# Tesla-Albert/Hybrid-Grid-for-Hexagonal-and-Rectangular-Image-Processing

Measured on AMD Instinct MI355X. Metric: Mpix/s rect→hex→rect+hexconv, 4K batch=128, 1/2/4/8 GPU; %HBM roofline, higher is better.
Workload: dtype bf16

## Files before the change

hybrid-grid-for-hexagonal-and-rectangular-image-processing_amd/csrc/fused4.hip:

```cpp
#include <climits>
#include <cmath>
#include <cstdlib>

#include "fused_kernel.h"

namespace hg {

#ifndef F4_RB_
#define F4_RB_ 30
#endif
#ifndef F4_PD
#define F4_PD 2
#endif
#ifndef F4_WPS
#define F4_WPS 29
#endif
#ifndef F4_ORDER
#define F4_ORDER 0
#endif
#ifndef F4_WPE
#define F4_WPE 3
#endif
#ifndef F4_REV
#define F4_REV 1
#endif
constexpr int F4_GW = 4, F4_THREADS = 256;
constexpr int F4_HL = 8, F4_OWN = 240;
constexpr int F4_RB = F4_RB_;
static_assert(F4_RB % 6 == 0 && F4_RB > 0, "bands are whole 6-step blocks");

typedef unsigned f4_u2 __attribute__((ext_vector_type(2)));

__device__ __forceinline__ void f4_unpack(f4_u2 r, fu_f2& a, fu_f2& b, unsigned hi16) {
    a = fu_f2{__builtin_bit_cast(float, r.x << 16), __builtin_bit_cast(float, r.x & hi16)};
    b = fu_f2{__builtin_bit_cast(float, r.y << 16), __builtin_bit_cast(float, r.y & hi16)};
}

template <int OP>
__global__ __launch_bounds__(F4_THREADS) __attribute__((amdgpu_waves_per_eu(F4_WPE)))
void k_fused4(const __bf16* __restrict__ x, const float* __restrict__ kern,
              const float* __restrict__ bias, __bf16* __restrict__ y, FusedGeom F) {
    constexpr int C = 3, O = 3;
    constexpr int PD = F4_PD;
    static_assert(PD >= 1 && PD <= 4, "raw ring: rows k+2 .. k+1+PD in flight in 6 slots");
    constexpr int RB = F4_RB, NLUT = RB + 2;
    __shared__ float4 lut_all[F4_GW][NLUT];
    const int lane = threadIdx.x & 63;
    const int wslot = __builtin_amdgcn_readfirstlane(threadIdx.x >> 6);
    float4* const lut = lut_all[wslot];
    const int64_t blk = (int64_t)xcd_swizzle(blockIdx.x, gridDim.x);
    const int ngrp = (F.nwin + F4_GW - 1) / F4_GW;
    const int grp = (int)(F4_ORDER == 1 ? (blk / F.nband) % ngrp : blk % ngrp);
    const int band = (int)(F4_ORDER == 1 ? blk % F.nband : (blk / ngrp) % F.nband);
    const int64_t b = blk / ((int64_t)ngrp * F.nband);
    if (b >= F.B) return;
    const int win = grp * F4_GW + wslot;
    const int W0 = win * F4_OWN - F4_HL;
    const int ce = W0 + 4 * lane;
    const int s0 = band * RB;
    const int s1 = min(s0 + RB, F.h2);
    const bool up = F4_REV && (band & 1) && s1 - s0 == RB;

    for (int e = lane; e < NLUT; e += 64) {
        const int r = s0 - 1 + e;
        float4 t = {0.f, 0.f, 0.f, 0.f};
        if (r >= 0 && r < F.h1) {
            const double i_ = axis_at(F.rxs, r) + (double)(F.h - 1) * 0.5;
            const int in = (int)i_;
            const double f = i_ - (double)(float)in;
            const float w0 = (in >= 0 && in < F.h) ? (float)(1.0 - f) : 0.f;
            const float w1 = (in + 1 >= 0 && in + 1 < F.h) ? (float)f : 0.f;
            if (in == r - 1) { t.x = w0; t.y = w1; }
            else if (in == r) { t.y = w0; t.z = w1; }
        }
        lut[e] = t;
    }
    __builtin_amdgcn_s_waitcnt(0xc07f);
    __builtin_amdgcn_wave_barrier();
    int rc;
    {
        bool has_a = false, has_c = false;
        for (int e = lane; e < NLUT; e += 64) {
            const float4 t = lut[e];
            has_a |= t.x != 0.f;
            has_c |= t.z != 0.f;
        }
        const bool any_a = __builtin_amdgcn_ballot_w64(has_a) != 0;
        const bool any_c = __builtin_amdgcn_ballot_w64(has_c) != 0;
        rc = !any_c ? 1 : (!any_a ? 2 : 0);
    }

    float we[2][3], wo[2][3];
#pragma unroll
    for (int k = 0; k < 2; ++k)
#pragma unroll
        for (int s = 0; s < 2; ++s) {
            float* wr = s ? wo[k] : we[k];
            wr[0] = wr[1] = wr[2] = 0.f;
            const int q = ce + 2 * k + s;
            if (q >= 0 && q < F.w1) {
                const double j_ = axis_at(F.rys, q) + (double)(F.w - 1) * 0.5;
                const int jn = (int)j_;
                const double jf = j_ - (double)(float)jn;
#pragma unroll
                for (int kk = -1; kk <= 1; ++kk) {
                    const bool in_w = q + kk >= 0 && q + kk < F.w;
                    if (kk == jn - q && in_w) wr[kk + 1] += (float)(1.0 - jf);
                    if (kk == jn + 1 - q && in_w) wr[kk + 1] += (float)jf;
                }
            }
#pragma unroll
            for (int t = 0; t < 3; ++t) wr[t] *= 0.75f;
        }
    const bool any_l = __builtin_amdgcn_ballot_w64(we[0][0] != 0.f || wo[0][0] != 0.f ||
                                                   we[1][0] != 0.f || wo[1][0] != 0.f) != 0;
    const bool any_r = __builtin_amdgcn_ballot_w64(we[0][2] != 0.f || wo[0][2] != 0.f ||
                                                   we[1][2] != 0.f || wo[1][2] != 0.f) != 0;
    const int cd = !any_r ? 1 : (!any_l ? 2 : 0);

    const bool own = lane >= F4_HL / 4 && lane < (F4_HL + F4_OWN) / 4 && ce >= 0 && ce < F.w2 &&
                     win < F.nwin;

    const int64_t cstride = (int64_t)F.h * F.w, ostride = (int64_t)F.h2 * F.w2;
    const __amdgpu_buffer_rsrc_t xrs = __builtin_amdgcn_make_buffer_rsrc(
        (void*)(x + b * C * cstride), (short)0, (int)(C * cstride * 2), 0x00020000);
    const __amdgpu_buffer_rsrc_t yrs = __builtin_amdgcn_make_buffer_rsrc(
        (void*)(y + b * O * ostride), (short)0, (int)(O * ostride * 2), 0x00020000);
    const int lc = min(max(ce, 0), F.w - 4);
    const unsigned xoff = (unsigned)lc * 2u;
    const unsigned yoff = own ? (unsigned)ce * 2u : 0x80000000u;
    const unsigned xplane = (unsigned)(cstride * 2), yplane = (unsigned)(ostride * 2);
    const unsigned xrow = (unsigned)F.w * 2u, yrow = (unsigned)F.w2 * 2u;
    auto row_off = [&](int r) -> unsigned {
        return (unsigned)__builtin_amdgcn_readfirstlane((int)((unsigned)min(max(r, 0), F.h - 1) * xrow));
    };

    int vz = 0;
    asm volatile("" : "+v"(vz));
    constexpr int NW = O * C * 7, NWP = (NW + 1) / 2;
    constexpr int NWS = F4_WPS < NWP ? F4_WPS : NWP;
    float wk[NW];
#pragma unroll
    for (int i = 0; i < NW; ++i) wk[i] = kern[i + (i / 2 < NWS ? 0 : vz)];
    fu_f2 wkp[NWP];
#pragma unroll
    for (int i = 0; i < NWP; ++i) {
        wkp[i] = fu_f2{wk[2 * i], 2 * i + 1 < NW ? wk[2 * i + 1] : 0.f};
        if (i >= NWS) asm volatile("" : "+v"(wkp[i]));
    }
    float bv[O];
#pragma unroll
    for (int o = 0; o < O; ++o) bv[o] = bias ? bias[o + vz] * 0.75f : 0.f;
    fu_f2 bvp[2];
#pragma unroll
    for (int i = 0; i < 2; ++i) {
        bvp[i] = fu_f2{bv[2 * i], 2 * i + 1 < O ? bv[2 * i + 1] : 0.f};
        asm volatile("" : "+v"(bvp[i]));
    }
    float c13 = 1.f / 3.f;
    asm volatile("" : "+v"(c13));
    const float wn_f = (ce + 4 < F.w2) ? c13 : 0.f;
    const float wp_f = (ce - 1 >= 0) ? c13 : 0.f;
    unsigned hi16 = 0xffff0000u;
    asm volatile("" : "+v"(hi16));

    auto run = [&](auto CDc, auto RCc, auto UPc) {
        constexpr int CD = decltype(CDc)::value;
        constexpr int RC = decltype(RCc)::value;
        constexpr bool UP = decltype(UPc)::value;
        auto row = [&](int k) { return UP ? s1 - 1 - k : s0 + k; };
        auto lut_e = [&](int j) { return UP ? RB - j : j + 1; };
        f4_u2 raw[6][C];
        fu_f2 XA[3][C], XB[3][C];
        fu_f2 ZA[3][O], ZB[3][O];

        auto issue = [&](auto SLc, int r, bool live = true) {
            constexpr int SL = decltype(SLc)::value;
            const unsigned so = row_off(r);
            const unsigned vo = live ? xoff : 0x80000000u;
#pragma unroll
            for (int c = 0; c < C; ++c) raw[SL][c] = __builtin_amdgcn_raw_buffer_load_b64(xrs, vo, so + c * xplane, 0);
        };
        auto convert = [&](auto RSc, auto XSc) {
            constexpr int RS = decltype(RSc)::value, XS = decltype(XSc)::value;
#pragma unroll
            for (int c = 0; c < C; ++c) f4_unpack(raw[RS][c], XA[XS][c], XB[XS][c], hi16);
        };

        auto urow = [&](auto PHc, float4 L, auto CENc, auto BELc) {
            constexpr int PH = decltype(PHc)::value;
            constexpr bool CEN = decltype(CENc)::value, BEL = decltype(BELc)::value;
            constexpr int S0 = fu_mod(PH, 3), S1 = fu_mod(PH + 1, 3), S2 = fu_mod(PH + 2, 3);
            constexpr int XM = UP ? S2 : S0, XQ = UP ? S0 : S2;
            constexpr int PB = UP ? fu_mod(PH + 1, 2) : fu_mod(PH, 2), PC = 1 - PB;
            constexpr int TN = UP ? 5 : 0, TD = UP ? 0 : 5;
            const fu_f2 Lxy = {L.x, L.y}, Lzw = {L.z, L.w};
            fu_sfor<0, C>([&](auto Cc) {
                constexpr int c = decltype(Cc)::value;
                float ue[2], uo[2];
                auto vblend = [&](const fu_f2 (&X)[3][C]) {
                    if constexpr (RC == 1) return fu_pfma<1, false>(Lxy, X[S1][c], fu_pmul<0>(Lxy, X[XM][c]));
                    else if constexpr (RC == 2) return fu_pfma<0, false>(Lzw, X[XQ][c], fu_pmul<1>(Lxy, X[S1][c]));
                    else return fu_pfma<0, false>(Lzw, X[XQ][c], fu_pfma<1, false>(Lxy, X[S1][c], fu_pmul<0>(Lxy, X[XM][c])));
                };
                const fu_f2 VA = vblend(XA), VB = vblend(XB);
                if constexpr (CD == 1) {
                    ue[0] = fmaf(we[0][1], VA.x, we[0][0] * f_prev(VB.y));
                    uo[0] = fmaf(wo[0][1], VA.y, wo[0][0] * VA.x);
                    ue[1] = fmaf(we[1][1], VB.x, we[1][0] * VA.y);
                    uo[1] = fmaf(wo[1][1], VB.y, wo[1][0] * VB.x);
                } else if constexpr (CD == 2) {
                    ue[0] = fmaf(we[0][2], VA.y, we[0][1] * VA.x);
                    uo[0] = fmaf(wo[0][2], VB.x, wo[0][1] * VA.y);
                    ue[1] = fmaf(we[1][2], VB.y, we[1][1] * VB.x);
                    uo[1] = fmaf(wo[1][2], f_next(VA.x), wo[1][1] * VB.y);
                } else {
                    const float pl = f_prev(VB.y), nx = f_next(VA.x);
                    ue[0] = fmaf(we[0][2], VA.y, fmaf(we[0][1], VA.x, we[0][0] * pl));
                    uo[0] = fmaf(wo[0][2], VB.x, fmaf(wo[0][1], VA.y, wo[0][0] * VA.x));
                    ue[1] = fmaf(we[1][2], VB.y, fmaf(we[1][1], VB.x, we[1][0] * VA.y));
                    uo[1] = fmaf(wo[1][2], nx, fmaf(wo[1][1], VB.y, wo[1][0] * VB.x));
                }
                const float nue = f_next(ue[0]);
                const fu_f2 U0[2] = {fu_f2{ue[0], uo[0]}, fu_f2{ue[1], uo[1]}};
                const fu_f2 U1[2] = {fu_f2{uo[0], ue[1]}, fu_f2{uo[1], nue}};
                const fu_f2 Um[2] = {fu_f2{f_prev(uo[1]), ue[0]}, fu_f2{uo[0], ue[1]}};
                const fu_f2 U2[2] = {U0[1], fu_f2{nue, OP == 0 ? f_next(uo[0]) : 0.f}};
                fu_sfor<0, O>([&](auto OOc) {
                    constexpr int o = decltype(OOc)::value;
                    constexpr int j0 = (o * C + c) * 7;
                    auto tapk = [&](auto Tc, fu_f2& zA, fu_f2& zB, int par) {
                        constexpr int j = j0 + decltype(Tc)::value;
                        constexpr bool WS = (j >> 1) < NWS;
                        const int s = fu_tap_shift(decltype(Tc)::value, par, OP);
                        const fu_f2 aA = s == -1 ? Um[0] : (s == 0 ? U0[0] : (s == 1 ? U1[0] : U2[0]));
                        const fu_f2 aB = s == -1 ? Um[1] : (s == 0 ? U0[1] : (s == 1 ? U1[1] : U2[1]));
                        zA = fu_pfma<j & 1, WS>(wkp[j >> 1], aA, zA);
                        zB = fu_pfma<j & 1, WS>(wkp[j >> 1], aB, zB);
                    };
                    if constexpr (c == 0) {
                        constexpr int jb = j0 + TN;
                        constexpr bool WS = (jb >> 1) < NWS;
                        const int s = fu_tap_shift(TN, PB, OP);
                        const fu_f2 aA = s == -1 ? Um[0] : (s == 0 ? U0[0] : (s == 1 ? U1[0] : U2[0]));
                        const fu_f2 aB = s == -1 ? Um[1] : (s == 0 ? U0[1] : (s == 1 ? U1[1] : U2[1]));
                        ZA[S2][o] = fu_pfma_b<jb & 1, o & 1, WS>(wkp[jb >> 1], aA, bvp[o >> 1]);
                        ZB[S2][o] = fu_pfma_b<jb & 1, o & 1, WS>(wkp[jb >> 1], aB, bvp[o >> 1]);
                    } else {
                        tapk(IC<TN>{}, ZA[S2][o], ZB[S2][o], PB);
                    }
                    tapk(IC<TN + 1>{}, ZA[S2][o], ZB[S2][o], PB);
                    if constexpr (CEN) {
                        tapk(IC<2>{}, ZA[S1][o], ZB[S1][o], PC);
                        tapk(IC<3>{}, ZA[S1][o], ZB[S1][o], PC);
                        tapk(IC<4>{}, ZA[S1][o], ZB[S1][o], PC);
                    }
                    if constexpr (BEL) {
                        tapk(IC<TD>{}, ZA[S0][o], ZB[S0][o], PB);
                        tapk(IC<TD + 1>{}, ZA[S0][o], ZB[S0][o], PB);
                    }
                });
            });
        };

        auto out_row = [&](auto PHc, int k) {
            constexpr int PH = decltype(PHc)::value;
            constexpr int S0 = PH % 3;
            constexpr int PAR = UP ? (PH + 1) & 1 : PH & 1;
            const unsigned so = (unsigned)__builtin_amdgcn_readfirstlane((int)((unsigned)row(k) * yrow));
#pragma unroll
            for (int o = 0; o < O; ++o) {
                const fu_f2 zA = ZA[S0][o], zB = ZB[S0][o];
                float o0, o1, o2, o3;
                if constexpr (PAR == 0) {
                    o0 = fmaf(c13, zA.y, zA.x);
                    o1 = fmaf(c13, zB.x, zA.y);
                    o2 = fmaf(c13, zB.y, zB.x);
                    o3 = fmaf(wn_f, f_next(zA.x), zB.y);
                } else {
                    o0 = fmaf(wp_f, f_prev(zB.y), zA.x);
                    o1 = fmaf(c13, zA.x, zA.y);
                    o2 = fmaf(c13, zA.y, zB.x);
                    o3 = fmaf(c13, zB.x, zB.y);
                }
                typedef __bf16 t2v __attribute__((ext_vector_type(2)));
                const f4_u2 v = {__builtin_bit_cast(unsigned, t2v{(__bf16)o0, (__bf16)o1}),
                                 __builtin_bit_cast(unsigned, t2v{(__bf16)o2, (__bf16)o3})};
                __builtin_amdgcn_raw_buffer_store_b64(v, yrs, yoff, so + o * yplane, 0);
            }
        };

        {
            f4_u2 t0[C], t1[C], t2[C];
            const unsigned o0 = row_off(row(-2)), o1 = row_off(row(-1)), o2 = row_off(row(0));
#pragma unroll
            for (int c = 0; c < C; ++c) {
                t0[c] = __builtin_amdgcn_raw_buffer_load_b64(xrs, xoff, o0 + c * xplane, 0);
                t1[c] = __builtin_amdgcn_raw_buffer_load_b64(xrs, xoff, o1 + c * xplane, 0);
                t2[c] = __builtin_amdgcn_raw_buffer_load_b64(xrs, xoff, o2 + c * xplane, 0);
            }
            issue(IC<1>{}, row(1));
#pragma unroll
            for (int i = 0; i < PD; ++i) {
                if (i == 0) issue(IC<2>{}, row(2));
                if (i == 1) issue(IC<3>{}, row(3));
                if (i == 2) issue(IC<4>{}, row(4));
                if (i == 3) issue(IC<5>{}, row(5));
            }
#pragma unroll
            for (int c = 0; c < C; ++c) {
                f4_unpack(t0[c], XA[1][c], XB[1][c], hi16);
                f4_unpack(t1[c], XA[2][c], XB[2][c], hi16);
                f4_unpack(t2[c], XA[0][c], XB[0][c], hi16);
            }
        }
        urow(IC<-2>{}, lut[lut_e(-1)], std::false_type{}, std::false_type{});
        convert(IC<1>{}, IC<1>{});
        urow(IC<-1>{}, lut[lut_e(0)], std::true_type{}, std::false_type{});
        __builtin_amdgcn_s_waitcnt(0x0f70);

        const int n = s1 - s0;
        float4 lnext = lut[lut_e(1)];
        auto step = [&](auto PHc, int k) {
            constexpr int PH = decltype(PHc)::value;
            __builtin_amdgcn_sched_barrier(0);
            convert(IC<(PH + 2) % 6>{}, IC<(PH + 2) % 3>{});
            issue(IC<(PH + 2 + PD) % 6>{}, row(min(k + 2 + PD, n + 1)), k + 2 + PD <= n + 1);
            const float4 L = lnext;
            lnext = lut[min(max(lut_e(k + 2), 0), NLUT - 1)];
            urow(PHc, L, std::true_type{}, std::true_type{});
            out_row(PHc, k);
        };
        auto block6 = [&](int base) {
            step(IC<0>{}, base);
            step(IC<1>{}, base + 1);
            step(IC<2>{}, base + 2);
            step(IC<3>{}, base + 3);
            step(IC<4>{}, base + 4);
            step(IC<5>{}, base + 5);
        };
        int base = 0;
        for (; base + 6 <= n; base += 6) block6(base);
        if constexpr (!UP) {
            if (base < n) {
                step(IC<0>{}, base);
                if (base + 1 < n) {
                    step(IC<1>{}, base + 1);
                    if (base + 2 < n) {
                        step(IC<2>{}, base + 2);
                        if (base + 3 < n) {
                            step(IC<3>{}, base + 3);
                            if (base + 4 < n) step(IC<4>{}, base + 4);
                        }
                    }
                }
            }
        }
    };
    auto dir = [&](auto CDc, auto RCc) {
        if (F4_REV && up) run(CDc, RCc, std::true_type{});
        else run(CDc, RCc, std::false_type{});
    };
    if (cd == 1 && rc == 1) dir(IC<1>{}, IC<1>{});
    else if (cd == 1 && rc == 2) dir(IC<1>{}, IC<2>{});
    else if (cd == 2 && rc == 1) dir(IC<2>{}, IC<1>{});
    else if (cd == 2 && rc == 2) dir(IC<2>{}, IC<2>{});
    else dir(IC<0>{}, IC<0>{});
}

int fused4_try(const void* x, const float* k, const float* bias, void* y, int x_dtype, int y_dtype,
               int C, int O, int G, const FusedGeom& F0, int op, hipStream_t st) {
    if (env_is("HYGRID_FUSED4", "0")) return HG_EUNSUP;
    if (x_dtype != HG_BF16 || y_dtype != HG_BF16 || C != 3 || O != 3 || G != 1) return HG_EUNSUP;
    if ((F0.w % 4) || (F0.w2 % 4) || F0.w < 4) return HG_EUNSUP;
    FusedGeom F = F0;
    F.nwin = (int)((F.w2 + F4_OWN - 1) / F4_OWN);
    F.nband = (int)((F.h2 + F4_RB - 1) / F4_RB);
    const int64_t blocks = F.B * (int64_t)F.nband * ((F.nwin + F4_GW - 1) / F4_GW);
    if (blocks > INT_MAX) return HG_EUNSUP;
    const dim3 grid((unsigned)blocks), blk(F4_THREADS);
    if (op)
        hipLaunchKernelGGL((k_fused4<1>), grid, blk, 0, st, (const __bf16*)x, k, bias, (__bf16*)y, F);
    else
        hipLaunchKernelGGL((k_fused4<0>), grid, blk, 0, st, (const __bf16*)x, k, bias, (__bf16*)y, F);
    return launch_status();
}

}

namespace hg {
void fused4_layout(int* band_rows, int* win_own, int* win_halo) {
    *band_rows = F4_RB;
    *win_own = F4_OWN;
    *win_halo = F4_HL;
}
}
```

Baseline: 401,900.

## Add optional persistent grid-stride loop to fused4 kernel and retune weight preload count

Restructures the fused4 kernel into a grid-stride loop over virtual blocks. Arguments are read through the kernarg segment pointer, and column state is cached across iterations that share the same window group. An opt-in persistent mode sizes the grid to the resident block count from an occupancy query, aiming to cut block launch and setup overhead. The number of preloaded weight pairs is also lowered from 29 to 26, which shifts register pressure. By default the grid stays at one block per tile, so the loop adds only a small overhead.

```diff
diff --git a/hybrid-grid-for-hexagonal-and-rectangular-image-processing_amd/csrc/fused4.hip b/hybrid-grid-for-hexagonal-and-rectangular-image-processing_amd/csrc/fused4.hip
--- a/hybrid-grid-for-hexagonal-and-rectangular-image-processing_amd/csrc/fused4.hip
+++ b/hybrid-grid-for-hexagonal-and-rectangular-image-processing_amd/csrc/fused4.hip
@@ -1,3 +1,5 @@
+#include <algorithm>
+#include <atomic>
 #include <climits>
 #include <cmath>
 #include <cstdlib>
@@ -13,7 +15,7 @@
 #define F4_PD 2
 #endif
 #ifndef F4_WPS
-#define F4_WPS 29
+#define F4_WPS 26
 #endif
 #ifndef F4_ORDER
 #define F4_ORDER 0
@@ -23,6 +25,9 @@
 #endif
 #ifndef F4_REV
 #define F4_REV 1
+#endif
+#ifndef F4_RESYNC
+#define F4_RESYNC 0
 #endif
 constexpr int F4_GW = 4, F4_THREADS = 256;
 constexpr int F4_HL = 8, F4_OWN = 240;
@@ -36,49 +41,50 @@
     b = fu_f2{__builtin_bit_cast(float, r.y << 16), __builtin_bit_cast(float, r.y & hi16)};
 }
 
+struct F4Args {
+    const __bf16* x;
+    const float* kern;
+    const float* bias;
+    __bf16* y;
+    FusedGeom F;
+    unsigned nblk, nslot;
+};
+__device__ __forceinline__ const F4Args* f4_args() {
+    auto kp = __builtin_amdgcn_kernarg_segment_ptr();
+    asm volatile("" : "+s"(kp));
+    return (const F4Args*)kp;
+}
+
 template <int OP>
 __global__ __launch_bounds__(F4_THREADS) __attribute__((amdgpu_waves_per_eu(F4_WPE)))
-void k_fused4(const __bf16* __restrict__ x, const float* __restrict__ kern,
-              const float* __restrict__ bias, __bf16* __restrict__ y, FusedGeom F) {
+void k_fused4(F4Args) {
     constexpr int C = 3, O = 3;
     constexpr int PD = F4_PD;
     static_assert(PD >= 1 && PD <= 4, "raw ring: rows k+2 .. k+1+PD in flight in 6 slots");
     constexpr int RB = F4_RB, NLUT = RB + 2;
     __shared__ float4 lut_all[F4_GW][NLUT];
-    const int lane = threadIdx.x & 63;
-    const int wslot = __builtin_amdgcn_readfirstlane(threadIdx.x >> 6);
+    int lane = threadIdx.x & 63;
+    const int wslot = threadIdx.x >> 6;
     float4* const lut = lut_all[wslot];
-    const int64_t blk = (int64_t)xcd_swizzle(blockIdx.x, gridDim.x);
-    const int ngrp = (F.nwin + F4_GW - 1) / F4_GW;
-    const int grp = (int)(F4_ORDER == 1 ? (blk / F.nband) % ngrp : blk % ngrp);
-    const int band = (int)(F4_ORDER == 1 ? blk % F.nband : (blk / ngrp) % F.nband);
-    const int64_t b = blk / ((int64_t)ngrp * F.nband);
-    if (b >= F.B) return;
-    const int win = grp * F4_GW + wslot;
-    const int W0 = win * F4_OWN - F4_HL;
-    const int ce = W0 + 4 * lane;
-    const int s0 = band * RB;
-    const int s1 = min(s0 + RB, F.h2);
-    const bool up = F4_REV && (band & 1) && s1 - s0 == RB;
-
-    for (int e = lane; e < NLUT; e += 64) {
-        const int r = s0 - 1 + e;
-        float4 t = {0.f, 0.f, 0.f, 0.f};
-        if (r >= 0 && r < F.h1) {
-            const double i_ = axis_at(F.rxs, r) + (double)(F.h - 1) * 0.5;
-            const int in = (int)i_;
-            const double f = i_ - (double)(float)in;
-            const float w0 = (in >= 0 && in < F.h) ? (float)(1.0 - f) : 0.f;
-            const float w1 = (in + 1 >= 0 && in + 1 < F.h) ? (float)f : 0.f;
-            if (in == r - 1) { t.x = w0; t.y = w1; }
-            else if (in == r) { t.y = w0; t.z = w1; }
-        }
-        lut[e] = t;
-    }
-    __builtin_amdgcn_s_waitcnt(0xc07f);
-    __builtin_amdgcn_wave_barrier();
-    int rc;
-    {
+    int s0 = 0, s1 = 0, hh = 0;
+
+    auto row_table = [&](const FusedGeom& F) -> int {
+        for (int e = lane; e < NLUT; e += 64) {
+            const int r = s0 - 1 + e;
+            float4 t = {0.f, 0.f, 0.f, 0.f};
+            if (r >= 0 && r < F.h1) {
+                const double i_ = axis_at(F.rxs, r) + (double)(F.h - 1) * 0.5;
+                const int in = (int)i_;
+                const double f = i_ - (double)(float)in;
+                const float w0 = (in >= 0 && in < F.h) ? (float)(1.0 - f) : 0.f;
+                const float w1 = (in + 1 >= 0 && in + 1 < F.h) ? (float)f : 0.f;
+                if (in == r - 1) { t.x = w0; t.y = w1; }
+                else if (in == r) { t.y = w0; t.z = w1; }
+            }
+            lut[e] = t;
+        }
+        __builtin_amdgcn_s_waitcnt(0xc07f);
+        __builtin_amdgcn_wave_barrier();
         bool has_a = false, has_c = false;
         for (int e = lane; e < NLUT; e += 64) {
             const float4 t = lut[e];
@@ -87,54 +93,65 @@
         }
         const bool any_a = __builtin_amdgcn_ballot_w64(has_a) != 0;
         const bool any_c = __builtin_amdgcn_ballot_w64(has_c) != 0;
-        rc = !any_c ? 1 : (!any_a ? 2 : 0);
-    }
-
-    float we[2][3], wo[2][3];
-#pragma unroll
-    for (int k = 0; k < 2; ++k)
-#pragma unroll
-        for (int s = 0; s < 2; ++s) {
-            float* wr = s ? wo[k] : we[k];
-            wr[0] = wr[1] = wr[2] = 0.f;
-            const int q = ce + 2 * k + s;
-            if (q >= 0 && q < F.w1) {
-                const double j_ = axis_at(F.rys, q) + (double)(F.w - 1) * 0.5;
-                const int jn = (int)j_;
-                const double jf = j_ - (double)(float)jn;
-#pragma unroll
-                for (int kk = -1; kk <= 1; ++kk) {
-                    const bool in_w = q + kk >= 0 && q + kk < F.w;
-                    if (kk == jn - q && in_w) wr[kk + 1] += (float)(1.0 - jf);
-                    if (kk == jn + 1 - q && in_w) wr[kk + 1] += (float)jf;
+        return !any_c ? 1 : (!any_a ? 2 : 0);
+    };
+
+    float c13 = 1.f / 3.f;
+    asm volatile("" : "+v"(c13));
+
+    float we[2][3] = {}, wo[2][3] = {};
+    int cd = 0;
+    unsigned xoff = 0, yoff = 0x80000000u;
+    float wn_f = 0.f, wp_f = 0.f;
+    auto col_state = [&](const FusedGeom& F, int grp) {
+        const int win = grp * F4_GW + wslot;
+        const int W0 = win * F4_OWN - F4_HL;
+        const int ce = W0 + 4 * lane;
+#pragma unroll
+        for (int k = 0; k < 2; ++k)
+#pragma unroll
+            for (int s = 0; s < 2; ++s) {
+                float* wr = s ? wo[k] : we[k];
+                wr[0] = wr[1] = wr[2] = 0.f;
+                const int q = ce + 2 * k + s;
+                if (q >= 0 && q < F.w1) {
+                    const double j_ = axis_at(F.rys, q) + (double)(F.w - 1) * 0.5;
+                    const int jn = (int)j_;
+                    const double jf = j_ - (double)(float)jn;
+#pragma unroll
+                    for (int kk = -1; kk <= 1; ++kk) {
+                        const bool in_w = q + kk >= 0 && q + kk < F.w;
+                        if (kk == jn - q && in_w) wr[kk + 1] += (float)(1.0 - jf);
+                        if (kk == jn + 1 - q && in_w) wr[kk + 1] += (float)jf;
+                    }
                 }
-            }
-#pragma unroll
-            for (int t = 0; t < 3; ++t) wr[t] *= 0.75f;
-        }
-    const bool any_l = __builtin_amdgcn_ballot_w64(we[0][0] != 0.f || wo[0][0] != 0.f ||
-                                                   we[1][0] != 0.f || wo[1][0] != 0.f) != 0;
-    const bool any_r = __builtin_amdgcn_ballot_w64(we[0][2] != 0.f || wo[0][2] != 0.f ||
-                                                   we[1][2] != 0.f || wo[1][2] != 0.f) != 0;
-    const int cd = !any_r ? 1 : (!any_l ? 2 : 0);
-
-    const bool own = lane >= F4_HL / 4 && lane < (F4_HL + F4_OWN) / 4 && ce >= 0 && ce < F.w2 &&
-                     win < F.nwin;
-
-    const int64_t cstride = (int64_t)F.h * F.w, ostride = (int64_t)F.h2 * F.w2;
-    const __amdgpu_buffer_rsrc_t xrs = __builtin_amdgcn_make_buffer_rsrc(
-        (void*)(x + b * C * cstride), (short)0, (int)(C * cstride * 2), 0x00020000);
-    const __amdgpu_buffer_rsrc_t yrs = __builtin_amdgcn_make_buffer_rsrc(
-        (void*)(y + b * O * ostride), (short)0, (int)(O * ostride * 2), 0x00020000);
-    const int lc = min(max(ce, 0), F.w - 4);
-    const unsigned xoff = (unsigned)lc * 2u;
-    const unsigned yoff = own ? (unsigned)ce * 2u : 0x80000000u;
-    const unsigned xplane = (unsigned)(cstride * 2), yplane = (unsigned)(ostride * 2);
-    const unsigned xrow = (unsigned)F.w * 2u, yrow = (unsigned)F.w2 * 2u;
+#pragma unroll
+                for (int t = 0; t < 3; ++t) wr[t] *= 0.75f;
+            }
+        const bool any_l = __builtin_amdgcn_ballot_w64(we[0][0] != 0.f || wo[0][0] != 0.f ||
+                                                       we[1][0] != 0.f || wo[1][0] != 0.f) != 0;
+        const bool any_r = __builtin_amdgcn_ballot_w64(we[0][2] != 0.f || wo[0][2] != 0.f ||
+                                                       we[1][2] != 0.f || wo[1][2] != 0.f) != 0;
+        cd = !any_r ? 1 : (!any_l ? 2 : 0);
+        const bool own = lane >= F4_HL / 4 && lane < (F4_HL + F4_OWN) / 4 && ce >= 0 &&
+                         ce < F.w2 && win < F.nwin;
+        const int lc = min(max(ce, 0), F.w - 4);
+        xoff = (unsigned)lc * 2u;
+        yoff = own ? (unsigned)ce * 2u : 0x80000000u;
+        wn_f = (ce + 4 < F.w2) ? c13 : 0.f;
+        wp_f = (ce - 1 >= 0) ? c13 : 0.f;
+    };
+
+    __amdgpu_buffer_rsrc_t xrs = __builtin_amdgcn_make_buffer_rsrc((void*)nullptr, (short)0, 0, 0x00020000);
+    __amdgpu_buffer_rsrc_t yrs = xrs;
+    unsigned xplane = 0, yplane = 0, xrow = 0, yrow = 0;
     auto row_off = [&](int r) -> unsigned {
-        return (unsigned)__builtin_amdgcn_readfirstlane((int)((unsigned)min(max(r, 0), F.h - 1) * xrow));
+        return (unsigned)__builtin_amdgcn_readfirstlane((int)((unsigned)min(max(r, 0), hh - 1) * xrow));
     };
 
+    typedef const float __attribute__((address_space(4)))* cfp;
+    const cfp kern = (cfp)f4_args()->kern;
+    const cfp bias = (cfp)f4_args()->bias;
     int vz = 0;
     asm volatile("" : "+v"(vz));
     constexpr int NW = O * C * 7, NWP = (NW + 1) / 2;
@@ -157,10 +174,6 @@
         bvp[i] = fu_f2{bv[2 * i], 2 * i + 1 < O ? bv[2 * i + 1] : 0.f};
         asm volatile("" : "+v"(bvp[i]));
     }
-    float c13 = 1.f / 3.f;
-    asm volatile("" : "+v"(c13));
-    const float wn_f = (ce + 4 < F.w2) ? c13 : 0.f;
-    const float wp_f = (ce - 1 >= 0) ? c13 : 0.f;
     unsigned hi16 = 0xffff0000u;
     asm volatile("" : "+v"(hi16));
 
@@ -357,15 +370,66 @@
             }
         }
     };
-    auto dir = [&](auto CDc, auto RCc) {
-        if (F4_REV && up) run(CDc, RCc, std::true_type{});
-        else run(CDc, RCc, std::false_type{});
-    };
-    if (cd == 1 && rc == 1) dir(IC<1>{}, IC<1>{});
-    else if (cd == 1 && rc == 2) dir(IC<1>{}, IC<2>{});
-    else if (cd == 2 && rc == 1) dir(IC<2>{}, IC<1>{});
-    else if (cd == 2 && rc == 2) dir(IC<2>{}, IC<2>{});
-    else dir(IC<0>{}, IC<0>{});
+
+    int cur_grp = -1;
+    for (unsigned vb = blockIdx.x;; vb += f4_args()->nslot) {
+        const F4Args* const A = f4_args();
+        const FusedGeom& F = A->F;
+        asm volatile("" : "+v"(lane));
+        const unsigned nblk = A->nblk;
+        if (vb >= nblk) break;
+        const int ngrp = (F.nwin + F4_GW - 1) / F4_GW;
+        const int64_t blk = (int64_t)xcd_swizzle(vb, nblk);
+        const int grp = (int)(F4_ORDER == 1 ? (blk / F.nband) % ngrp : blk % ngrp);
+        const int band = (int)(F4_ORDER == 1 ? blk % F.nband : (blk / ngrp) % F.nband);
+        const int64_t b = blk / ((int64_t)ngrp * F.nband);
+        if (grp != cur_grp) {
+            col_state(F, grp);
+            cur_grp = grp;
+        }
+#if F4_RESYNC
+        __builtin_amdgcn_s_barrier();
+#endif
+        s0 = band * RB;
+        s1 = min(s0 + RB, F.h2);
+        hh = F.h;
+        const bool up = F4_REV && (band & 1) && s1 - s0 == RB;
+        const int rc = row_table(F);
+        const int64_t cstride = (int64_t)F.h * F.w, ostride = (int64_t)F.h2 * F.w2;
+        xplane = (unsigned)(cstride * 2), yplane = (unsigned)(ostride * 2);
+        xrow = (unsigned)F.w * 2u, yrow = (unsigned)F.w2 * 2u;
+        xrs = __builtin_amdgcn_make_buffer_rsrc(
+            (void*)(A->x + b * C * cstride), (short)0, (int)(C * cstride * 2), 0x00020000);
+        yrs = __builtin_amdgcn_make_buffer_rsrc(
+            (void*)(A->y + b * O * ostride), (short)0, (int)(O * ostride * 2), 0x00020000);
+        auto dir = [&](auto CDc, auto RCc) {
+            if (F4_REV && up) run(CDc, RCc, std::true_type{});
+            else run(CDc, RCc, std::false_type{});
+        };
+        if (cd == 1 && rc == 1) dir(IC<1>{}, IC<1>{});
+        else if (cd == 1 && rc == 2) dir(IC<1>{}, IC<2>{});
+        else if (cd == 2 && rc == 1) dir(IC<2>{}, IC<1>{});
+        else if (cd == 2 && rc == 2) dir(IC<2>{}, IC<2>{});
+        else dir(IC<0>{}, IC<0>{});
+    }
+}
+
+template <int OP>
+static int f4_resident() {
+    static std::atomic<int> cache[64];
+    int dev = 0;
+    if (hipGetDevice(&dev) != hipSuccess || dev < 0 || dev >= 64) return 0;
+    int v = cache[dev].load(std::memory_order_relaxed);
+    if (v == 0) {
+        int cus = 0, per_cu = 0;
+        if (hipDeviceGetAttribute(&cus, hipDeviceAttributeMultiprocessorCount, dev) != hipSuccess ||
+            hipOccupancyMaxActiveBlocksPerMultiprocessor(&per_cu, k_fused4<OP>, F4_THREADS, 0) != hipSuccess)
+            cus = per_cu = 0;
+        (void)hipGetLastError();
+        v = cus > 0 && per_cu > 0 ? cus * per_cu : -1;
+        cache[dev].store(v, std::memory_order_relaxed);
+    }
+    return v > 0 ? v : 0;
 }
 
 int fused4_try(const void* x, const float* k, const float* bias, void* y, int x_dtype, int y_dtype,
@@ -378,11 +442,24 @@
     F.nband = (int)((F.h2 + F4_RB - 1) / F4_RB);
     const int64_t blocks = F.B * (int64_t)F.nband * ((F.nwin + F4_GW - 1) / F4_GW);
     if (blocks > INT_MAX) return HG_EUNSUP;
-    const dim3 grid((unsigned)blocks), blk(F4_THREADS);
+    int64_t slots = blocks;
+    if (env_is("HYGRID_F4_PERSIST", "1")) {
+        const char* e = getenv("HYGRID_F4_SLOTS");
+        const long forced = e ? strtol(e, nullptr, 10) : 0;
+        if (forced > 0) {
+            slots = std::min<int64_t>(forced, blocks);
+        } else {
+            const int64_t res = op ? f4_resident<1>() : f4_resident<0>();
+            const int64_t unit = 8 * (int64_t)((F.nwin + F4_GW - 1) / F4_GW);
+            if (res > 0 && res < blocks) slots = res >= unit ? res / unit * unit : res;
+        }
+    }
+    const dim3 grid((unsigned)slots), blk(F4_THREADS);
+    const F4Args A = {(const __bf16*)x, k, bias, (__bf16*)y, F, (unsigned)blocks, (unsigned)slots};
     if (op)
-        hipLaunchKernelGGL((k_fused4<1>), grid, blk, 0, st, (const __bf16*)x, k, bias, (__bf16*)y, F);
+        hipLaunchKernelGGL((k_fused4<1>), grid, blk, 0, st, A);
     else
-        hipLaunchKernelGGL((k_fused4<0>), grid, blk, 0, st, (const __bf16*)x, k, bias, (__bf16*)y, F);
+        hipLaunchKernelGGL((k_fused4<0>), grid, blk, 0, st, A);
     return launch_status();
 }
 
```

After: 401,000. Within noise of the previous version (-0.2%).
